# dluvizon/deephar

Hardware: NVIDIA H100
Metric: frames/sec (256x256, 16-frame clips, b32) (higher is better)
Workload: dtype bf16x3 split (fp32 accumulate, wgmma)

## Files before the change

deephar_b200/_ffi.py:

```python
import ctypes as C
import os

_HERE = os.path.dirname(os.path.abspath(__file__))
LIB_PATH = os.environ.get('DEEPHAR_B200_LIB') or os.path.join(_HERE, 'libdeephar_b200.so')


class DeepharB200Error(RuntimeError):
    pass


class dh_view(C.Structure):
    _fields_ = [('p', C.c_void_p), ('n', C.c_int32), ('h', C.c_int32), ('w', C.c_int32),
                ('c', C.c_int32), ('ld', C.c_int32)]


class dh_conv_desc(C.Structure):
    _fields_ = [('kh', C.c_int32), ('kw', C.c_int32), ('sh', C.c_int32), ('sw', C.c_int32),
                ('pad_same', C.c_int32), ('pre_relu', C.c_int32), ('post_relu', C.c_int32),
                ('n_res', C.c_int32),
                ('pre_scale', C.c_void_p), ('pre_shift', C.c_void_p),
                ('post_scale', C.c_void_p), ('post_shift', C.c_void_p),
                ('res', dh_view * 2),
                ('precision', C.c_int32), ('res_up2x', C.c_int32), ('pool_out', dh_view)]


class dh_frame_src(C.Structure):
    _fields_ = [('data', C.c_uint64), ('h', C.c_int32), ('w', C.c_int32), ('stride', C.c_int32),
                ('x0', C.c_int32), ('y0', C.c_int32), ('cw', C.c_int32), ('ch', C.c_int32), ('hflip', C.c_int32),
                ('kx_off', C.c_int32), ('ky_off', C.c_int32), ('kx_coef_off', C.c_int32), ('ky_coef_off', C.c_int32),
                ('ksx', C.c_int32), ('ksy', C.c_int32)]


class dh_packed_w(C.Structure):
    _fields_ = [('hi', C.c_void_p), ('lo', C.c_void_p), ('cout_pad', C.c_int32), ('k', C.c_int32)]


class dh_conv_plan_info(C.Structure):
    _fields_ = [('path', C.c_int32), ('fallback', C.c_int32), ('workspace_bytes', C.c_int64),
                ('n_mtiles', C.c_int32), ('grid_x', C.c_int32), ('grid_y', C.c_int32), ('bn_cta', C.c_int32),
                ('n_kblocks', C.c_int32), ('stages', C.c_int32), ('cluster', C.c_int32), ('bm', C.c_int32),
                ('epi_tma', C.c_int32)]


class dh_clip_window(C.Structure):
    _fields_ = [('src', dh_view), ('dst', dh_view), ('ring', C.c_void_p)]


class dh_jpeg_image(C.Structure):
    _fields_ = [('data', C.c_int64), ('coef', C.c_int64 * 3), ('plane', C.c_int64 * 3), ('out', C.c_int64),
                ('h', C.c_int32), ('w', C.c_int32), ('ncomp', C.c_int32), ('hs', C.c_int32), ('vs', C.c_int32),
                ('mcus_x', C.c_int32), ('mcus_y', C.c_int32), ('bw', C.c_int32 * 3), ('bh', C.c_int32 * 3),
                ('qt', C.c_int32 * 3), ('dc', C.c_int32 * 3), ('ac', C.c_int32 * 3), ('nblocks', C.c_int32),
                ('pad', C.c_int32)]


class dh_jpeg_segment(C.Structure):
    _fields_ = [('begin', C.c_int64), ('end', C.c_int64), ('image', C.c_int32), ('mcu0', C.c_int32),
                ('mcus', C.c_int32), ('pad', C.c_int32)]


class dh_jpeg_huff(C.Structure):
    _fields_ = [('lut', C.c_uint16 * 512), ('maxcode', C.c_int32 * 18), ('valoff', C.c_int32 * 18),
                ('vals', C.c_uint8 * 256)]

# ... 144 lines not shown
```

deephar_b200/csrc/api.cu:

```cuda
#include <stdarg.h>
#include <string.h>
#include "common.cuh"

static thread_local char g_last_error[512] = "";

void dh_set_error(const char* fmt, ...) {
    va_list ap;
    va_start(ap, fmt);
    vsnprintf(g_last_error, sizeof(g_last_error), fmt, ap);
    va_end(ap);
}

extern "C" const char* dh_last_error(void) { return g_last_error; }

extern "C" int dh_version(void) { return 100; }

extern "C" int dh_ctx_create(dh_ctx** out, int device) {
    DH_CHECK_ARG(out != nullptr, "dh_ctx_create: out is NULL");
    int count = 0;
    cudaError_t e = cudaGetDeviceCount(&count);
    if (e != cudaSuccess || count == 0) {
        dh_set_error("dh_ctx_create: no CUDA device (%s) -- this library has no CPU fallback",
                     cudaGetErrorString(e));
        return e == cudaSuccess ? (int)cudaErrorNoDevice : (int)e;
    }
    DH_CHECK_ARG(device >= 0 && device < count, "dh_ctx_create: device %d out of range", device);
    cudaDeviceProp prop;
    e = cudaGetDeviceProperties(&prop, device);
    if (e != cudaSuccess) {
        dh_set_error("cudaGetDeviceProperties: %s", cudaGetErrorString(e));
        return (int)e;
    }
    if (prop.major != 9 || prop.minor != 0) {
        dh_set_error("dh_ctx_create: device %d is sm_%d%d; this build targets sm_90a (H100) only",
                     device, prop.major, prop.minor);
        return -2;
    }
    dh_ctx* c = new dh_ctx();
    c->device = device;
    c->num_sms = prop.multiProcessorCount;
    c->launches = 0;
    c->workspace = nullptr;
    c->workspace_bytes = 0;
    c->last_conv_path = 0;
    c->share_a = 1;
    c->sep_tma = 1;
    c->dbg = 0;
    c->pw_smallk = 1;
    c->dense_patch = 1;
    c->sam3d_stream = 1;
    c->fallbacks = 0;
    c->comm = nullptr;
    c->comm_rank = -1;
    c->comm_world = 0;
    *out = c;
    return 0;
}

extern "C" int dh_comm_destroy(dh_ctx* ctx);

extern "C" int dh_ctx_destroy(dh_ctx* ctx) {
    if (ctx && ctx->comm) dh_comm_destroy(ctx);
    delete ctx;
    return 0;
}

extern "C" int64_t dh_launch_count(dh_ctx* ctx, int reset) {
    if (!ctx) return -1;
    int64_t v = ctx->launches;
    if (reset) ctx->launches = 0;
    return v;
}

extern "C" int dh_set_option(dh_ctx* ctx, const char* name, int value) {
    DH_CHECK_ARG(ctx && name, "dh_set_option: NULL argument");
    if (!strcmp(name, "share_a")) { ctx->share_a = value; return 0; }
    if (!strcmp(name, "sep_tma")) { ctx->sep_tma = value; return 0; }
#ifdef DH_ABLATE
    if (!strcmp(name, "dbg")) { ctx->dbg = value; return 0; }
#endif
    if (!strcmp(name, "pw_smallk")) { ctx->pw_smallk = value; return 0; }
    if (!strcmp(name, "dense_patch")) { ctx->dense_patch = value; return 0; }
    if (!strcmp(name, "sam3d_stream")) { ctx->sam3d_stream = value; return 0; }
    dh_set_error("dh_set_option: unknown option %s", name);
    return -1;
}

extern "C" int dh_last_conv_path(dh_ctx* ctx) { return ctx ? ctx->last_conv_path : -1; }

extern "C" int64_t dh_fallback_count(dh_ctx* ctx, int reset) {
    if (!ctx) return -1;
    int64_t v = ctx->fallbacks;
    if (reset) ctx->fallbacks = 0;
    return v;
}

extern "C" int dh_set_workspace(dh_ctx* ctx, void* ptr, int64_t bytes) {
    DH_CHECK_ARG(ctx != nullptr, "dh_set_workspace: ctx is NULL");
    ctx->workspace = ptr;
    ctx->workspace_bytes = bytes;
// ... 3 lines not shown
```

deephar_b200/csrc/common.cuh:

```cuda
#pragma once
#include <cuda_runtime.h>
#include <stdint.h>
#include <stdio.h>
#include "../../include/deephar_b200.h"

struct dh_ctx {
    int device;
    int num_sms;
    int64_t launches;
    void* workspace;
    int64_t workspace_bytes;
    int last_conv_path;
    int share_a;
    int sep_tma;
    int pw_smallk;
    int sam3d_stream;
    int dense_patch;
    void* comm;
    int comm_rank, comm_world;
    int64_t fallbacks;
    int dbg;
};

void dh_set_error(const char* fmt, ...);

#define DH_CHECK_ARG(cond, ...)            \
    do {                                   \
        if (!(cond)) {                     \
            dh_set_error(__VA_ARGS__);     \
            return -1;                     \
        }                                  \
    } while (0)

#define DH_LAUNCH_EPILOGUE(ctx, nlaunch)                     \
    do {                                                     \
        (ctx)->launches += (nlaunch);                        \
        cudaError_t e__ = cudaGetLastError();                \
// ... 97 lines not shown
```

deephar_b200/csrc/conv_api.cu:

```cuda
#include "tc_common.cuh"

namespace {

struct Choice {
    DhConvPath path;
    bool fallback;
    int64_t workspace_bytes;
    tc::PatchPlan patch;
    tc::SepPlan sep;
    tc::TcPlan tcp;
};

int choose_conv(const dh_ctx* ctx, const ConvParams& p, const dh_packed_w* packed, bool separable, int precision,
                Choice* c) {
    const bool packed_hi = packed && packed->hi;
    c->fallback = false;
    c->workspace_bytes = 0;
    if (separable) {
        DH_CHECK_ARG(!p.pool, "dh_sepconv2d_f32: pool_out is not supported by the separable kernels");
        if (packed_hi && dh_plan_sep_tma(ctx, p, packed, precision, &c->sep)) { c->path = DH_PATH_SEP_TMA; return 0; }
    } else {
        if (!p.up1 && !p.pool && dh_conv_smallk_ok(p)) { c->path = DH_PATH_SIMT; return 0; }
        if (ctx->pw_smallk && !p.up1 && dh_pw_smallk_supported(p)) { c->path = DH_PATH_PW_SMALLK; return 0; }
        DH_CHECK_ARG(!p.pool, "dh_conv2d_f32: pool_out is written by the wide pointwise kernel only (1x1, stride 1, "
// ... 56 lines not shown
    info->n_mtiles = P.n_mtiles;
    info->grid_x = tc::persistent_gx(ctx, pl.gy, P.n_mtiles);
    info->grid_y = pl.gy;
    info->bn_cta = P.bn_cta;
    info->n_kblocks = P.n_kblocks;
    info->cluster = pl.cluster;
    info->bm = tc::BM;
}

int plan_info(const dh_ctx* ctx, const Choice& c, dh_conv_plan_info* info) {
    DH_CHECK_ARG(info, "dh_conv_plan_info: NULL info");
    *info = dh_conv_plan_info{};
    info->path = c.path;
    info->fallback = c.fallback;
    info->workspace_bytes = c.workspace_bytes;
    if (c.path == DH_PATH_TC) {
        tc_info(ctx, c.tcp, c.tcp.k, info);
        info->stages = c.tcp.k.stages;
    }
    if (c.path == DH_PATH_SEP_TMA) {
        tc_info(ctx, c.sep, c.sep.k.t, info);
        info->bm = c.sep.k.bm;
        info->epi_tma = c.sep.k.epi_smem > 0;
    }
    if (c.path == DH_PATH_PATCH) tc_info(ctx, c.patch, c.patch.k.t, info);
    return 0;
}

}

extern "C" int dh_conv2d_f32(dh_ctx* ctx, const dh_view* x, const float* w_hwio,
                             const dh_packed_w* packed, const dh_conv_desc* d, const dh_view* out,
                             void* stream) {
    ConvParams p;
    Choice c;
    int rc = plan_conv(ctx, x, nullptr, w_hwio, packed, d, out, false, &p, &c);
    return rc ? rc : launch_choice(ctx, p, c, false, (cudaStream_t)stream);
}

extern "C" int dh_sepconv2d_f32(dh_ctx* ctx, const dh_view* x, const float* w_dw, const float* w_pw,
                                const dh_packed_w* packed_pw, const dh_conv_desc* d,
                                const dh_view* out, void* stream) {
    ConvParams p;
    Choice c;
    int rc = plan_conv(ctx, x, w_dw, w_pw, packed_pw, d, out, true, &p, &c);
    return rc ? rc : launch_choice(ctx, p, c, true, (cudaStream_t)stream);
// ... 19 lines not shown
```

deephar_b200/csrc/conv_sep.cu:

```cuda
#include "tc_common.cuh"

namespace tcs {
using namespace tc;
using R = tc::Roles<2, 1>;
constexpr int WARP_EPI0 = R::WARP_EPI0, WARP_TMA = R::WARP_TMA, WARP_PATCH = R::WARP_PATCH, NTHREADS = R::NTHREADS,
              REGS_PROD = R::REGS_PROD, REGS_EPI = R::REGS_EPI, REGS_CTRL = R::REGS_CTRL;

constexpr int NWG = 128;
constexpr int NPW = 1;
constexpr int NA = 4;
constexpr int NB = 3;
constexpr int NP = 3;
#ifdef DH_ABLATE
constexpr int DBG_TILE64 = 1 << 14, DBG_TILE128 = 1 << 15;
constexpr int DBG_EPI_REG = 1 << 16;
#endif

template <int TBM, int KS, int TW, bool SHARE, bool BNPRO, bool LO>
__global__ void __launch_bounds__(NTHREADS, 1)
sep_tma_kernel(const __grid_constant__ SepParams SP, const __grid_constant__ CUtensorMap map_hi,
               const __grid_constant__ CUtensorMap map_lo, const __grid_constant__ CUtensorMap map_x,
               const __grid_constant__ CUtensorMap map_out, const __grid_constant__ CUtensorMap map_r0,
               const __grid_constant__ CUtensorMap map_r1) {
    constexpr int PAD = KS / 2;
    constexpr int PC = TW + 2 * PAD;
    constexpr int OR = TBM / 32;
    constexpr int NR = OR + KS - 1;
    constexpr int NC = 4 + KS - 1;
    constexpr int A_BYTES = TBM * 64;
#ifdef DH_ABLATE
    const int DBG = SP.dbg;
#else
    constexpr int DBG = 0;
#endif
    const TcParams& P = SP.t;
    extern __shared__ __align__(1024) uint8_t smem_raw[];
    if (smem_u32(smem_raw) & 1023u) __trap();
    uint8_t* smem = smem_raw;
    const int tid = threadIdx.x;
    const int warp = tid >> 5, lane = tid & 31;
    constexpr bool want_lo = LO;
    const int b_bytes = P.bn_cta * 64;
    uint8_t* b_ring = smem + NA * 2 * A_BYTES;
    uint8_t* patch0 = b_ring + NB * 2 * b_bytes;
    uint8_t* epi_buf = patch0 + NP * SP.patch_stride;
    uint64_t* bars = reinterpret_cast<uint64_t*>(epi_buf + SP.epi_smem);
    float* post = reinterpret_cast<float*>(bars + 64);
    constexpr int NB_A = NA + 2 * NA;
    const uint32_t bar_full0 = smem_u32(bars), bar_empty0 = smem_u32(bars + NA), bar_fullb0 = smem_u32(bars + NB_A),
                   bar_emptyb0 = smem_u32(bars + NB_A + NB), bar_pfull0 = smem_u32(bars + NB_A + 2 * NB),
                   bar_pempty0 = smem_u32(bars + NB_A + 2 * NB + NP), bar_epi_full0 = smem_u32(bars + NB_A + 2 * NB + 2 * NP),
                   bar_epi_empty = bar_epi_full0 + 16;
    const bool epi = TBM == BM64 && SP.epi_smem > 0;
    const int n0 = blockIdx.y * P.bn_cta;
    const int nkb = P.n_kblocks;
    const uint32_t my_rank = SHARE ? cluster_ctarank() : 0u;

    if (warp == WARP_TMA && lane == 0) {
        tma_prefetch_desc(&map_hi);
        if (want_lo) tma_prefetch_desc(&map_lo);
        tma_prefetch_desc(&map_x);
        if (epi) {
            tma_prefetch_desc(&map_out);
            mbar_init(bar_epi_full0, 1);
            mbar_init(bar_epi_full0 + 8, 1);
            mbar_init(bar_epi_empty, 1);
        }
        for (int s = 0; s < NA; ++s) {
            mbar_init(bar_full0 + 8 * s, SHARE ? 1u : (uint32_t)NWG);
            const uint32_t releases = SHARE && (uint32_t)(s & 1) == my_rank ? 2u : 1u;
            mbar_init(bar_empty0 + 16 * s, releases);
            mbar_init(bar_empty0 + 16 * s + 8, releases);
        }
        for (int s = 0; s < NB; ++s) {
            mbar_init(bar_fullb0 + 8 * s, 1);
            mbar_init(bar_emptyb0 + 8 * s, 1);
        }
        for (int s = 0; s < NP; ++s) {
            mbar_init(bar_pfull0 + 8 * s, 1);
            mbar_init(bar_pempty0 + 8 * s, NWG);
        }
        fence_barrier_init();
    }
    if (SHARE) cluster_sync_all(); else __syncthreads();

    const int tiles_mine = ((int)P.n_mtiles - (int)blockIdx.x + (int)gridDim.x - 1) / (int)gridDim.x;
    const int total_g = tiles_mine * nkb;
    const int n_own = SHARE ? (total_g - (int)my_rank + 1) / 2 : total_g;

    if (warp < WARP_EPI0) {
        reg_prod<REGS_PROD, R::LAUNCH_REGS>();
        const ConvParams& c = P.c;
        const int w = warp >> 2;
        const int tw = tid & (NWG - 1);
        const int cp = tw & 15;
        const int blk = tw >> 4;
        constexpr int XB = TW / 4;
        const int strip = blk / XB, xb = blk - strip * XB;
        const int fn = (strip * OR) / SP.ry, ry = (strip * OR) - fn * SP.ry;
        const int prr = SP.ry + 2 * PAD;
        const float* pbase0 = reinterpret_cast<const float*>(patch0) +
                             ((size_t)((fn * prr + ry) * PC + xb * 4)) * SBK + cp * 2;
        const int row0 = strip * OR * TW + xb * 4;
        const float lowb = c.pre_relu ? 0.f : -3.402823466e38f;
        unsigned colmask = 0;
        if (BNPRO) {
#pragma unroll
            for (int q = 0; q < NC; ++q) {
                const int ix = xb * 4 + q - PAD;
                if (ix >= 0 && ix < TW) colmask |= 1u << q;
            }
        }
        float2 wt[KS][KS];
        auto load_taps = [&](int jn) {
            const int gn = SHARE ? 2 * jn + (int)my_rank : jn;
            const int kbn = gn % nkb;
            const float* wp = c.w_dw + kbn * SBK + cp * 2;
#pragma unroll
            for (int a = 0; a < KS; ++a)
#pragma unroll
                for (int b = 0; b < KS; ++b)
                    wt[a][b] = __ldg(reinterpret_cast<const float2*>(wp + (size_t)(a * KS + b) * c.Cin));
        };
        if (w < n_own) load_taps(w);
        for (int j = w; j < n_own; j += NPW) {
            const int pb_i = j % NP;
            const uint32_t pfull = bar_pfull0 + 8 * pb_i, pempty = bar_pempty0 + 8 * pb_i;
            const float* pbase = pbase0 + (size_t)pb_i * (SP.patch_stride / 4);
            const int g = SHARE ? 2 * j + (int)my_rank : j;
            const int ti = g / nkb, kb = g - ti * nkb;
            const int ch = kb * SBK + cp * 2;
            float2 acc[OR][4];
#pragma unroll
            for (int o = 0; o < OR; ++o)
#pragma unroll
                for (int q = 0; q < 4; ++q) acc[o][q] = make_float2(0.f, 0.f);
            float2 ps = make_float2(1.f, 1.f), pb = make_float2(0.f, 0.f);
            unsigned rowmask = 0;
            if (BNPRO) {
                ps = __ldg(reinterpret_cast<const float2*>(c.pre_scale + ch));
                pb = __ldg(reinterpret_cast<const float2*>(c.pre_shift + ch));
                const int t = blockIdx.x + ti * gridDim.x;
                const int y0 = SP.fn > 1 ? 0 : ((t * TBM) / TW) % c.H;
#pragma unroll
                for (int r = 0; r < NR; ++r) {
                    const int iy = y0 + ry + r - PAD;
                    if (iy >= 0 && iy < c.H) rowmask |= 1u << r;
                }
            }

            if (!(DBG & 2)) mbar_wait_relaxed(pfull, (uint32_t)((j / NP) & 1), (DBG & 2048) ? 32u : 0u);
            auto load_row = [&](int r, float2* in) {
#pragma unroll
                for (int q = 0; q < NC; ++q) {
                    float2 v = *reinterpret_cast<const float2*>(pbase + (r * PC + q) * SBK);
                    if (BNPRO) v = ffma2(v, ps, pb);
                    v = make_float2(fmaxf(v.x, lowb), fmaxf(v.y, lowb));
                    if (BNPRO && !(((rowmask >> r) & 1u) && ((colmask >> q) & 1u))) v = make_float2(0.f, 0.f);
                    in[q] = v;
                }
            };
            if (!(DBG & 1)) {
                float2 inb[2][NC];
                load_row(0, inb[0]);
#pragma unroll
                for (int r = 0; r < NR; ++r) {
                    if (r + 1 < NR) load_row(r + 1, inb[(r + 1) & 1]);
                    const float2* in = inb[r & 1];
#pragma unroll
                    for (int kx = 0; kx < KS; ++kx)
#pragma unroll
                        for (int o = 0; o < OR; ++o) {
                            const int ky = r - o;
                            if (ky >= 0 && ky < KS) {
#pragma unroll
                                for (int q = 0; q < 4; ++q) acc[o][q] = ffma2(wt[ky][kx], in[q + kx], acc[o][q]);
                            }
                        }
                }
            }
            if (j + NPW < n_own) load_taps(j + NPW);
            if (!(DBG & 2)) mbar_arrive(pempty);

            const int s = g % NA;
            const uint32_t it = (uint32_t)(g / NA);
            wait_stage_free(bar_empty0, s, it, (DBG & 2048) ? 32u : 0u);
            uint8_t* a_hi = smem + (size_t)s * (2 * A_BYTES);
            uint8_t* a_lo = a_hi + A_BYTES;
#pragma unroll
            for (int o = 0; o < OR; ++o)
#pragma unroll
                for (int q = 0; q < 4; ++q) {
                    uint32_t hi, lo;
                    split2(acc[o][q].x, acc[o][q].y, hi, lo);
                    const uint32_t off = swz64(row0 + o * TW + q, cp * 2);
                    *reinterpret_cast<uint32_t*>(a_hi + off) = hi;
                    if (want_lo) *reinterpret_cast<uint32_t*>(a_lo + off) = lo;
                }
            fence_proxy_async();
            if (SHARE) {
                asm volatile("bar.sync %0, %1;" ::"r"(1 + w), "r"(NWG) : "memory");
                if (tw == 0) {
                    mbar_arrive(bar_full0 + 8 * s);
                    const uint32_t peer = my_rank ^ 1u;
                    const uint32_t peer_full = mapa_peer(bar_full0 + 8 * s, peer);
                    if (!(DBG & 8)) {
                        bulk_s2peer(mapa_peer(smem_u32(a_hi), peer), smem_u32(a_hi), A_BYTES, peer_full);
                        if (want_lo) bulk_s2peer(mapa_peer(smem_u32(a_lo), peer), smem_u32(a_lo), A_BYTES, peer_full);
                    }
                }
            } else {
                mbar_arrive(bar_full0 + 8 * s);
            }
        }
    } else if (warp < WARP_TMA) {
        reg_inc<REGS_EPI>();
        stage_post<R::NEPI, bn_max(TBM)>(P, n0, post, tid - 32 * WARP_EPI0);
        const int wg = (warp - WARP_EPI0) >> 2, wt = tid - 32 * WARP_EPI0 - 128 * wg;
        const EpiSmem es{epi ? reinterpret_cast<float*>(epi_buf) : nullptr,
                         P.c.res1 ? reinterpret_cast<const float*>(epi_buf + EPI_BUF_BYTES) : nullptr, bar_epi_full0,
                         bar_epi_empty, &map_out};
        pp_consumer<SHARE, LO, NA, NB, TBM>(P, wg, wt, n0, tiles_mine, make_desc64(smem_u32(smem)), make_desc64(smem_u32(b_ring)),
                                       bar_full0, bar_empty0, bar_fullb0, bar_emptyb0, my_rank, post, DBG,
                                       es);
    } else {
        reg_dec<REGS_CTRL>();
        if (warp == WARP_TMA) {
            if (lane == 0) {
                const uint32_t tx = (DBG & 16) ? 0u : (uint32_t)(want_lo ? 2 : 1) * (uint32_t)b_bytes;
                const uint32_t tx_a = (DBG & 8) ? 0u : (uint32_t)(want_lo ? 2 : 1) * (uint32_t)A_BYTES;
                for (int g = 0; g < total_g; ++g) {
                    const int ti = g / nkb, kb = g - ti * nkb;
                    const int sb = g % NB;
                    const uint32_t itb = (uint32_t)(g / NB);
                    if (itb >= 1) mbar_wait_relaxed(bar_emptyb0 + 8 * sb, (itb - 1) & 1, (DBG & 2048) ? 64u : 0u);
                    const uint32_t full = bar_fullb0 + 8 * sb;
                    mbar_arrive_expect_tx(full, tx);
                    const uint32_t b_hi = smem_u32(b_ring + (size_t)sb * (2 * b_bytes));
                    const uint32_t b_lo = b_hi + (uint32_t)b_bytes;
                    if (!(DBG & 16)) {
                        tma_load_2d(b_hi, &map_hi, kb * SBK, n0, full);
                        if (want_lo) tma_load_2d(b_lo, &map_lo, kb * SBK, n0, full);
                    }
                    if (SHARE && (uint32_t)(g & 1) != my_rank) {
                        const int sa = g % NA;
                        wait_stage_free(bar_empty0, sa, (uint32_t)(g / NA));
                        mbar_arrive_expect_tx(bar_full0 + 8 * sa, tx_a);
                    }
                }
            }
        } else if (warp == WARP_TMA + 1) {
            if (lane == 0 && epi) {
                const ConvParams& c = P.c;
                const uint32_t tx = (DBG & 32) ? 0u
                                               : (c.res0 ? (uint32_t)EPI_BUF_BYTES : 0u) + (c.res1 ? (uint32_t)EPI_R1_BYTES : 0u);
                for (int ti = 0; ti < tiles_mine; ++ti) {
                    if (ti >= 1) mbar_wait_relaxed(bar_epi_empty, (uint32_t)((ti - 1) & 1), 0u);
                    const int m0 = ((int)blockIdx.x + ti * (int)gridDim.x) * TBM;
                    const uint32_t full = bar_epi_full0 + 8 * (ti & 1);
                    mbar_arrive_expect_tx(full, tx);
                    if (tx) {
                        if (c.res0) tma_load_2d(smem_u32(epi_buf), &map_r0, n0, m0, full);
                        if (c.res1) tma_load_2d(smem_u32(epi_buf + EPI_BUF_BYTES), &map_r1, n0, m0 / 4, full);
                    }
                }
            }
        } else if (warp == WARP_PATCH) {
            if (lane == 0 && !(DBG & 2)) {
                const ConvParams& c = P.c;
                auto coords = [&](int j, int& kb, int& nf, int& y0) {
                    const int g = SHARE ? 2 * j + (int)my_rank : j;
                    const int ti = g / nkb;
                    kb = g - ti * nkb;
                    const int t = blockIdx.x + ti * gridDim.x;
                    const int grow = (t * TBM) / TW;
                    nf = grow / c.H;
                    y0 = grow - nf * c.H;
                };
                for (int j = 0; j < n_own; ++j) {
                    int kb, nf, y0;
                    coords(j, kb, nf, y0);
                    const int w = j % NP;
                    const int pfd = (DBG & 1024) ? 2 : (DBG & 4096) ? 4 : (DBG & 8192) ? 9 : 0;
                    if (pfd && j + pfd < n_own) {
                        int kb2, nf2, y2;
                        coords(j + pfd, kb2, nf2, y2);
                        tma_prefetch_4d(&map_x, kb2 * SBK, -PAD, y2 - PAD, nf2);
                    }
                    mbar_wait_relaxed(bar_pempty0 + 8 * w, (uint32_t)(((j / NP) & 1) ^ 1), (DBG & 2048) ? 64u : 0u);
                    const uint32_t pf = bar_pfull0 + 8 * w;
                    mbar_arrive_expect_tx(pf, (uint32_t)SP.patch_bytes);
                    tma_load_4d(smem_u32(patch0 + (size_t)w * SP.patch_stride), &map_x, kb * SBK, -PAD, y0 - PAD, nf, pf);
                }
            }
        }
    }
    if (SHARE) cluster_sync_all(); else __syncthreads();
}

}

bool dh_plan_sep_tma(const dh_ctx* ctx, const ConvParams& p, const dh_packed_w* packed, int precision, tc::SepPlan* pl) {
    using namespace tc;
    using namespace tcs;
    if (!ctx->sep_tma || !packed->lo || !sep_layer_ok(p, packed)) return false;
    if (!(p.W == 32 || p.W == 16 || p.W == 8)) return false;
    const int tr = BM / p.W;
    if (tr <= p.H ? (p.H % tr) != 0 : (tr % p.H) != 0) return false;
    if ((p.Cin % SBK) != 0 || (p.ldx & 3)) return false;
    int bn64, gy64;
    tile_n(p.Cout, &bn64, &gy64, MAX_BN_CTA64);
    const bool fits64 = ctx->share_a && bn64 == MAX_BN_CTA64 && gy64 % 2 == 0;
    bool t64 = fits64 && p.Cin >= 288;
#ifdef DH_ABLATE
    if (ctx->dbg & DBG_TILE64) t64 = fits64;
    if (ctx->dbg & DBG_TILE128) t64 = false;
#endif
    SepParams& SP = pl->k;
    TcParams& P = SP.t;
    P.c = p;
    P.c.K = p.Cin;
    P.k_pad = packed->k;
    P.n_kblocks = p.Cin / SBK;
    P.precision = (precision == 1) ? 1 : 3;
    P.ks = p.kh;
    P.stages = 2;
    const int pad = p.kh / 2;
#ifdef DH_ABLATE
    SP.dbg = ctx->dbg;
    P.dbg = ctx->dbg;
#else
    SP.dbg = 0;
    P.dbg = 0;
#endif
    auto geometry = [&](int bm) {
        int gy;
        tile_n(p.Cout, &P.bn_cta, &gy, bn_max(bm));
        const int trb = bm / p.W;
        SP.bm = bm;
        P.n_mtiles = (p.M + bm - 1) / bm;
        SP.ry = trb <= p.H ? trb : p.H;
        SP.fn = trb <= p.H ? 1 : trb / p.H;
        SP.patch_bytes = SBK * 4 * (p.W + 2 * pad) * (SP.ry + 2 * pad) * SP.fn;
        SP.patch_stride = (SP.patch_bytes + 1023) / 1024 * 1024;
        pl->smem = (size_t)NA * 2 * (bm * 64) + (size_t)NB * 2 * P.bn_cta * 64 + NP * (size_t)SP.patch_stride + 512 +
                   post_smem(bm);
        pl->gy = gy;
        return pl->smem <= SMEM_LIMIT;
    };
    SP.epi_smem = 0;
    if (!(t64 && geometry(BM64)) && !geometry(BM)) return false;
    bool epi = SP.bm == BM64 && tma_view_ok(p.out, p.ldo) && (!p.res0 || tma_view_ok(p.res0, p.ldr0)) &&
               (!p.res1 || (p.up1 && tma_view_ok(p.res1, p.ldr1)));
#ifdef DH_ABLATE
    if (ctx->dbg & DBG_EPI_REG) epi = false;
#endif
    const int epi_smem = EPI_BUF_BYTES + (p.res1 ? EPI_R1_BYTES : 0);
    if (epi && pl->smem + epi_smem <= SMEM_LIMIT) {
        SP.epi_smem = epi_smem;
        pl->smem += epi_smem;
    }
    pl->w = packed;
    pl->cluster = pl->gy % 2 == 0 && ctx->share_a;
    return true;
}

int dh_launch_sep_tma(const dh_ctx* ctx, const tc::SepPlan& pl, cudaStream_t s) {
    using namespace tc;
    using namespace tcs;
    const TcParams& P = pl.k.t;
    const ConvParams& c = P.c;
    const dh_packed_w* w = pl.w;
    const int pad = P.ks / 2;
    CUtensorMap map_hi, map_lo, map_x, map_out{}, map_r0{}, map_r1{};
    const bool epi = pl.k.epi_smem > 0;
    if (!make_map_w(&map_hi, w->hi, w->k, w->cout_pad, SBK, P.bn_cta) ||
        !make_map_w(&map_lo, w->lo, w->k, w->cout_pad, SBK, P.bn_cta) ||
        !make_map_x(&map_x, c.x, c.ldx, c.Cin, c.W, c.H, c.N, c.W + 2 * pad, pl.k.ry + 2 * pad, pl.k.fn) ||
        (epi && !make_map_rows(&map_out, c.out, c.Cout, c.M, c.ldo, MAX_BN_CTA64, BM64)) ||
        (epi && c.res0 && !make_map_rows(&map_r0, c.res0, c.Cout, c.M, c.ldr0, MAX_BN_CTA64, BM64)) ||
        (epi && c.res1 && !make_map_rows(&map_r1, c.res1, c.Cout, c.M / 4, c.ldr1, MAX_BN_CTA64, BM64 / 4))) {
        dh_set_error("dh_launch_sep_tma: cuTensorMapEncodeTiled failed");
        return -1;
    }
    return pick<5, 3>(P.ks, [&](auto ks) {
        return pick<32, 16, 8>(c.W, [&](auto tw) {
            return pick<true, false>(c.pre_scale != nullptr, [&](auto bnpro) {
                return pick<true, false>(P.precision == 3, [&](auto lo) {
                    if (pl.k.bm == BM64)
                        return launch_persistent<sep_tma_kernel<BM64, ks(), tw(), true, bnpro(), lo()>>(
                            "dh_launch_sep_tma", ctx, pl, P.n_mtiles, NTHREADS, s, map_hi, map_lo, map_x, map_out, map_r0, map_r1);
                    return pick<true, false>(pl.cluster, [&](auto share) {
                        return launch_persistent<sep_tma_kernel<BM, ks(), tw(), share(), bnpro(), lo()>>(
                            "dh_launch_sep_tma", ctx, pl, P.n_mtiles, NTHREADS, s, map_hi, map_lo, map_x, map_out, map_r0, map_r1);
                    });
                });
            });
        });
    });
}
```

deephar_b200/csrc/tc_common.cuh:

```cuda
#pragma once
#include <cuda.h>
#include <cuda_bf16.h>
#include <type_traits>
#include "common.cuh"
#include "conv_params.cuh"

namespace tc {


constexpr int BM = 128;
constexpr int BK = 64;
constexpr int NPROD = 256;
constexpr int MAX_BN_CTA = 96;
constexpr int ACC_N = MAX_BN_CTA / 2;
constexpr int MH = BM / 64;
constexpr int BM64 = 64;
constexpr int MAX_BN_CTA64 = 144;
constexpr int bn_max(int bm) { return bm == BM64 ? MAX_BN_CTA64 : MAX_BN_CTA; }
template <int Q, int NPW = 2>
struct Roles {
    static constexpr int EPQ = Q;
    static constexpr int NEPI = 128 * Q;
    static constexpr int WARP_EPI0 = 4 * NPW;
    static constexpr int WARP_TMA = WARP_EPI0 + 4 * Q, WARP_PATCH = WARP_TMA + 2;
// ... 6 lines not shown
};
constexpr int A_TILE_BYTES = BM * 128;
constexpr int MAX_STAGES = 4;

struct TcParams {
    ConvParams c;
    int n_kblocks;
    int bn_cta;
    int stages;
    int precision;
    int ks;
    int k_pad;
    int n_mtiles;
    int dbg;
};

struct SepParams {
    TcParams t;
    int patch_stride;
    int patch_bytes;
    int ry, fn;
    int bm;
    int epi_smem;
    int dbg;
};

struct PatchParams {
    TcParams t;
    int np, patch_stride, patch_bytes;
    int ntaps, ncb;
    int tw;
    int ry, fn;
    int pc, pr;
    int rows_per_frame;
    int kw;
    int pt, pl, sh, sw;
    int vh, vw;
    int mask;
};

__device__ __forceinline__ void mbar_wait_relaxed(uint32_t bar, uint32_t parity, uint32_t ns) {
    uint32_t ok;
    for (;;) {
        asm volatile(
            "{\n .reg .pred p;\n mbarrier.try_wait.parity.shared::cta.b64 p, [%1], %2;\n selp.u32 %0, 1, 0, p;\n}"
            : "=r"(ok)
// ... 416 lines not shown
                const int g = g0 + kb, s = g % NA, sb = g % NB;
                if (!(dbg & 128)) mbar_wait(bar_full0 + 8 * s, (uint32_t)(g / NA) & 1);
                mbar_wait(bar_fullb0 + 8 * sb, (uint32_t)(g / NB) & 1);
                if (kb == nkb - 1 && ti + 1 < tiles_mine) pp_pass(wg);
                da = dbase + (uint64_t)((uint32_t)s * sta16);
                db = dbase_b + (uint64_t)((uint32_t)sb * stb16);
            },
            [&](int kb) {
                const int g = g0 + kb, s = g % NA;
                const uint32_t producer = (uint32_t)(s & 1);
                wg_release(bar_empty0 + 16 * s + 8 * ((g / NA) & 1), wg, wt, SHARE && producer != rank, producer);
                if (wt == 0) mbar_arrive(bar_emptyb0 + 8 * (g % NB));
            });
        if constexpr (TBM == BM64) {
            if (es.buf) {
                wg_epilogue_smem(P, acc, ti, m0, n0, wg, wt, post, es);
                continue;
            }
        }
        wg_epilogue(P, acc, m0, n0, wt, post);
    }
}

typedef CUresult (*EncodeTiledFn)(CUtensorMap*, CUtensorMapDataType, cuuint32_t, void*, const cuuint64_t*,
                                  const cuuint64_t*, const cuuint32_t*, const cuuint32_t*, CUtensorMapInterleave,
                                  CUtensorMapSwizzle, CUtensorMapL2promotion, CUtensorMapFloatOOBfill);

static inline EncodeTiledFn get_encode() {
    static EncodeTiledFn fn = nullptr;
    if (!fn) {
        void* p = nullptr;
        cudaDriverEntryPointQueryResult qres;
        if (cudaGetDriverEntryPoint("cuTensorMapEncodeTiled", &p, cudaEnableDefault, &qres) == cudaSuccess &&
            qres == cudaDriverEntryPointSuccess)
            fn = (EncodeTiledFn)p;
    }
    return fn;
}

static inline bool make_map_w(CUtensorMap* map, const void* base, int k_pad, int rows, int kblk, int box_rows) {
    EncodeTiledFn enc = get_encode();
    if (!enc) return false;
    cuuint64_t dims[2] = {(cuuint64_t)k_pad, (cuuint64_t)rows};
    cuuint64_t strides[1] = {(cuuint64_t)k_pad * 2};
    cuuint32_t box[2] = {(cuuint32_t)kblk, (cuuint32_t)box_rows};
    cuuint32_t estr[2] = {1, 1};
// ... 124 lines not shown
```

include/deephar_b200.h:

```cpp
#ifndef DEEPHAR_B200_H
#define DEEPHAR_B200_H

#include <stdint.h>

#ifdef __cplusplus
extern "C" {
#endif

typedef struct dh_view {
    float*  p;
    int32_t n, h, w, c;
    int32_t ld;
} dh_view;

typedef struct dh_conv_desc {
    int32_t kh, kw, sh, sw;
    int32_t pad_same;
    int32_t pre_relu;
    int32_t post_relu;
    int32_t n_res;
    const float* pre_scale;
    const float* pre_shift;
    const float* post_scale;
    const float* post_shift;
// ... 23 lines not shown
int dh_tc_k_pad(int k);
int dh_last_conv_path(dh_ctx* ctx);
int64_t dh_fallback_count(dh_ctx* ctx, int reset);

int dh_conv2d_f32(dh_ctx* ctx, const dh_view* x, const float* w_hwio, const dh_packed_w* packed,
                  const dh_conv_desc* d, const dh_view* out, void* stream);

int dh_sepconv2d_f32(dh_ctx* ctx, const dh_view* x, const float* w_dw, const float* w_pw,
                     const dh_packed_w* packed_pw, const dh_conv_desc* d, const dh_view* out,
                     void* stream);

typedef struct dh_conv_plan_info {
    int32_t path;
    int32_t fallback;
    int64_t workspace_bytes;
    int32_t n_mtiles;
    int32_t grid_x, grid_y;
    int32_t bn_cta;
    int32_t n_kblocks;
    int32_t stages;
    int32_t cluster;
    int32_t bm;
    int32_t epi_tma;
} dh_conv_plan_info;
int dh_conv2d_plan(dh_ctx* ctx, const dh_view* x, const float* w_hwio, const dh_packed_w* packed,
                   const dh_conv_desc* d, const dh_view* out, dh_conv_plan_info* info);
int dh_sepconv2d_plan(dh_ctx* ctx, const dh_view* x, const float* w_dw, const float* w_pw,
                      const dh_packed_w* packed_pw, const dh_conv_desc* d, const dh_view* out,
                      dh_conv_plan_info* info);

int dh_maxpool2d_f32(dh_ctx* ctx, const dh_view* x, int kh, int kw, int sh, int sw, int pad_same,
                     const dh_view* out, void* stream);
int dh_upsample2x_add_f32(dh_ctx* ctx, const dh_view* a, const dh_view* b, const dh_view* out,
                          void* stream);
int dh_add_n_f32(dh_ctx* ctx, const dh_view* in, int n_in, const float* scale, const float* shift,
                 int relu, const dh_view* out, void* stream);

int dh_softargmax2d_f32(dh_ctx* ctx, const dh_view* h, const dh_view* d, float alpha,
                        int conf_on_prob, float* out_pose, float* out_conf,
                        const dh_view* prob_out, void* stream);

int dh_softargmax2d_ctx_f32(dh_ctx* ctx, const dh_view* h, int nj, int n_ctx, float alpha_mix,
                            float* out_pose, float* out_vis, void* stream);

int dh_softargmax3d_f32(dh_ctx* ctx, const dh_view* h, int nj, int depth_maps,
                        float* out_pose, float* out_vis, void* stream);
// ... 150 lines not shown
```

Measured before the change: 4063.

## Co-schedule pairs of 64-row tiles in separable conv TMA kernel

Adds a co-scheduled mode to the separable-conv kernel. Each A stage now holds two 64-row M tiles, so the two consumer warpgroups each take one tile of the pair and share a single B-stage fetch. The goal is to halve the B-operand traffic and the per-k-block barrier overhead when there are many k-blocks. In exchange the A ring doubles in size and the patch ring shrinks to two buffers, and the mode is only chosen when there are enough k-blocks and the epilogue TMA views are valid.

Result: faster. 4204, median of 6 (+3.5%).

```diff
diff --git a/deephar_b200/_ffi.py b/deephar_b200/_ffi.py
--- a/deephar_b200/_ffi.py
+++ b/deephar_b200/_ffi.py
@@ -39,7 +39,7 @@
     _fields_ = [('path', C.c_int32), ('fallback', C.c_int32), ('workspace_bytes', C.c_int64),
                 ('n_mtiles', C.c_int32), ('grid_x', C.c_int32), ('grid_y', C.c_int32), ('bn_cta', C.c_int32),
                 ('n_kblocks', C.c_int32), ('stages', C.c_int32), ('cluster', C.c_int32), ('bm', C.c_int32),
-                ('epi_tma', C.c_int32)]
+                ('epi_tma', C.c_int32), ('cosched', C.c_int32)]
 
 
 class dh_clip_window(C.Structure):
diff --git a/deephar_b200/csrc/api.cu b/deephar_b200/csrc/api.cu
--- a/deephar_b200/csrc/api.cu
+++ b/deephar_b200/csrc/api.cu
@@ -45,6 +45,7 @@
     c->last_conv_path = 0;
     c->share_a = 1;
     c->sep_tma = 1;
+    c->sep_cosched = 1;
     c->dbg = 0;
     c->pw_smallk = 1;
     c->dense_patch = 1;
@@ -76,6 +77,7 @@
     DH_CHECK_ARG(ctx && name, "dh_set_option: NULL argument");
     if (!strcmp(name, "share_a")) { ctx->share_a = value; return 0; }
     if (!strcmp(name, "sep_tma")) { ctx->sep_tma = value; return 0; }
+    if (!strcmp(name, "sep_cosched")) { ctx->sep_cosched = value; return 0; }
 #ifdef DH_ABLATE
     if (!strcmp(name, "dbg")) { ctx->dbg = value; return 0; }
 #endif
diff --git a/deephar_b200/csrc/common.cuh b/deephar_b200/csrc/common.cuh
--- a/deephar_b200/csrc/common.cuh
+++ b/deephar_b200/csrc/common.cuh
@@ -13,6 +13,7 @@
     int last_conv_path;
     int share_a;
     int sep_tma;
+    int sep_cosched;
     int pw_smallk;
     int sam3d_stream;
     int dense_patch;
diff --git a/deephar_b200/csrc/conv_api.cu b/deephar_b200/csrc/conv_api.cu
--- a/deephar_b200/csrc/conv_api.cu
+++ b/deephar_b200/csrc/conv_api.cu
@@ -102,6 +102,7 @@
         tc_info(ctx, c.sep, c.sep.k.t, info);
         info->bm = c.sep.k.bm;
         info->epi_tma = c.sep.k.epi_smem > 0;
+        info->cosched = c.sep.k.cosched;
     }
     if (c.path == DH_PATH_PATCH) tc_info(ctx, c.patch, c.patch.k.t, info);
     return 0;
diff --git a/deephar_b200/csrc/conv_sep.cu b/deephar_b200/csrc/conv_sep.cu
--- a/deephar_b200/csrc/conv_sep.cu
+++ b/deephar_b200/csrc/conv_sep.cu
@@ -11,12 +11,18 @@
 constexpr int NA = 4;
 constexpr int NB = 3;
 constexpr int NP = 3;
+constexpr int NP_COS = 2;
+constexpr int COS_PATCH_MAX = SBK * 4 * (32 + 4) * (2 + 4);
+static_assert(NA * 4 * (BM64 * 64) + NB * 2 * (MAX_BN_CTA64 * 64) + NP_COS * COS_PATCH_MAX + EPI_BUF_BYTES +
+                  EPI_R1_BYTES + 512 + post_smem(BM64) <= SMEM_LIMIT,
+              "co-scheduled 64 x 144 rings do not fit at 5x5, W = 32, with an up2x residual");
+constexpr int COS_MIN_KBLOCKS = 12;
 #ifdef DH_ABLATE
 constexpr int DBG_TILE64 = 1 << 14, DBG_TILE128 = 1 << 15;
 constexpr int DBG_EPI_REG = 1 << 16;
 #endif
 
-template <int TBM, int KS, int TW, bool SHARE, bool BNPRO, bool LO>
+template <int TBM, int KS, int TW, bool SHARE, bool BNPRO, bool LO, bool COS>
 __global__ void __launch_bounds__(NTHREADS, 1)
 sep_tma_kernel(const __grid_constant__ SepParams SP, const __grid_constant__ CUtensorMap map_hi,
                const __grid_constant__ CUtensorMap map_lo, const __grid_constant__ CUtensorMap map_x,
@@ -28,6 +34,10 @@
     constexpr int NR = OR + KS - 1;
     constexpr int NC = 4 + KS - 1;
     constexpr int A_BYTES = TBM * 64;
+    static_assert(!COS || (TBM == BM64 && SHARE), "co-scheduling runs the 64-row tiles of cluster pairs");
+    constexpr int NH = COS ? 2 : 1;
+    constexpr int A_STAGE = NH * 2 * A_BYTES;
+    constexpr int NPB = COS ? NP_COS : NP;
 #ifdef DH_ABLATE
     const int DBG = SP.dbg;
 #else
@@ -41,16 +51,16 @@
     const int warp = tid >> 5, lane = tid & 31;
     constexpr bool want_lo = LO;
     const int b_bytes = P.bn_cta * 64;
-    uint8_t* b_ring = smem + NA * 2 * A_BYTES;
+    uint8_t* b_ring = smem + NA * A_STAGE;
     uint8_t* patch0 = b_ring + NB * 2 * b_bytes;
-    uint8_t* epi_buf = patch0 + NP * SP.patch_stride;
+    uint8_t* epi_buf = patch0 + NPB * SP.patch_stride;
     uint64_t* bars = reinterpret_cast<uint64_t*>(epi_buf + SP.epi_smem);
     float* post = reinterpret_cast<float*>(bars + 64);
     constexpr int NB_A = NA + 2 * NA;
     const uint32_t bar_full0 = smem_u32(bars), bar_empty0 = smem_u32(bars + NA), bar_fullb0 = smem_u32(bars + NB_A),
                    bar_emptyb0 = smem_u32(bars + NB_A + NB), bar_pfull0 = smem_u32(bars + NB_A + 2 * NB),
-                   bar_pempty0 = smem_u32(bars + NB_A + 2 * NB + NP), bar_epi_full0 = smem_u32(bars + NB_A + 2 * NB + 2 * NP),
-                   bar_epi_empty = bar_epi_full0 + 16;
+                   bar_pempty0 = smem_u32(bars + NB_A + 2 * NB + NPB),
+                   bar_epi_full0 = smem_u32(bars + NB_A + 2 * NB + 2 * NPB), bar_epi_empty = bar_epi_full0 + 16;
     const bool epi = TBM == BM64 && SP.epi_smem > 0;
     const int n0 = blockIdx.y * P.bn_cta;
     const int nkb = P.n_kblocks;
@@ -68,15 +78,15 @@
         }
         for (int s = 0; s < NA; ++s) {
             mbar_init(bar_full0 + 8 * s, SHARE ? 1u : (uint32_t)NWG);
-            const uint32_t releases = SHARE && (uint32_t)(s & 1) == my_rank ? 2u : 1u;
+            const uint32_t releases = (uint32_t)NH * (SHARE && (uint32_t)(s & 1) == my_rank ? 2u : 1u);
             mbar_init(bar_empty0 + 16 * s, releases);
             mbar_init(bar_empty0 + 16 * s + 8, releases);
         }
         for (int s = 0; s < NB; ++s) {
             mbar_init(bar_fullb0 + 8 * s, 1);
-            mbar_init(bar_emptyb0 + 8 * s, 1);
-        }
-        for (int s = 0; s < NP; ++s) {
+            mbar_init(bar_emptyb0 + 8 * s, NH);
+        }
+        for (int s = 0; s < NPB; ++s) {
             mbar_init(bar_pfull0 + 8 * s, 1);
             mbar_init(bar_pempty0 + 8 * s, NWG);
         }
@@ -85,7 +95,8 @@
     if (SHARE) cluster_sync_all(); else __syncthreads();
 
     const int tiles_mine = ((int)P.n_mtiles - (int)blockIdx.x + (int)gridDim.x - 1) / (int)gridDim.x;
-    const int total_g = tiles_mine * nkb;
+    const int total_g = (COS ? (tiles_mine + 1) / 2 : tiles_mine) * nkb;
+    auto tiles_of = [&](int u) { return COS && 2 * u + 1 < tiles_mine ? 2 : 1; };
     const int n_own = SHARE ? (total_g - (int)my_rank + 1) / 2 : total_g;
 
     if (warp < WARP_EPI0) {
@@ -123,80 +134,87 @@
                     wt[a][b] = __ldg(reinterpret_cast<const float2*>(wp + (size_t)(a * KS + b) * c.Cin));
         };
         if (w < n_own) load_taps(w);
+        int box = 0;
         for (int j = w; j < n_own; j += NPW) {
-            const int pb_i = j % NP;
-            const uint32_t pfull = bar_pfull0 + 8 * pb_i, pempty = bar_pempty0 + 8 * pb_i;
-            const float* pbase = pbase0 + (size_t)pb_i * (SP.patch_stride / 4);
             const int g = SHARE ? 2 * j + (int)my_rank : j;
-            const int ti = g / nkb, kb = g - ti * nkb;
+            const int u = g / nkb, kb = g - u * nkb;
+            const int nh = tiles_of(u);
             const int ch = kb * SBK + cp * 2;
-            float2 acc[OR][4];
-#pragma unroll
-            for (int o = 0; o < OR; ++o)
-#pragma unroll
-                for (int q = 0; q < 4; ++q) acc[o][q] = make_float2(0.f, 0.f);
             float2 ps = make_float2(1.f, 1.f), pb = make_float2(0.f, 0.f);
-            unsigned rowmask = 0;
             if (BNPRO) {
                 ps = __ldg(reinterpret_cast<const float2*>(c.pre_scale + ch));
                 pb = __ldg(reinterpret_cast<const float2*>(c.pre_shift + ch));
-                const int t = blockIdx.x + ti * gridDim.x;
-                const int y0 = SP.fn > 1 ? 0 : ((t * TBM) / TW) % c.H;
-#pragma unroll
-                for (int r = 0; r < NR; ++r) {
-                    const int iy = y0 + ry + r - PAD;
-                    if (iy >= 0 && iy < c.H) rowmask |= 1u << r;
-                }
-            }
-
-            if (!(DBG & 2)) mbar_wait_relaxed(pfull, (uint32_t)((j / NP) & 1), (DBG & 2048) ? 32u : 0u);
-            auto load_row = [&](int r, float2* in) {
-#pragma unroll
-                for (int q = 0; q < NC; ++q) {
-                    float2 v = *reinterpret_cast<const float2*>(pbase + (r * PC + q) * SBK);
-                    if (BNPRO) v = ffma2(v, ps, pb);
-                    v = make_float2(fmaxf(v.x, lowb), fmaxf(v.y, lowb));
-                    if (BNPRO && !(((rowmask >> r) & 1u) && ((colmask >> q) & 1u))) v = make_float2(0.f, 0.f);
-                    in[q] = v;
-                }
-            };
-            if (!(DBG & 1)) {
-                float2 inb[2][NC];
-                load_row(0, inb[0]);
-#pragma unroll
-                for (int r = 0; r < NR; ++r) {
-                    if (r + 1 < NR) load_row(r + 1, inb[(r + 1) & 1]);
-                    const float2* in = inb[r & 1];
-#pragma unroll
-                    for (int kx = 0; kx < KS; ++kx)
-#pragma unroll
-                        for (int o = 0; o < OR; ++o) {
-                            const int ky = r - o;
-                            if (ky >= 0 && ky < KS) {
-#pragma unroll
-                                for (int q = 0; q < 4; ++q) acc[o][q] = ffma2(wt[ky][kx], in[q + kx], acc[o][q]);
+            }
+            const int s = g % NA;
+            uint8_t* a_stage = smem + (size_t)s * A_STAGE;
+            for (int h = 0; h < nh; ++h, ++box) {
+                const int pb_i = box % NPB;
+                const uint32_t pfull = bar_pfull0 + 8 * pb_i, pempty = bar_pempty0 + 8 * pb_i;
+                const float* pbase = pbase0 + (size_t)pb_i * (SP.patch_stride / 4);
+                const int ti = COS ? 2 * u + h : u;
+                float2 acc[OR][4];
+#pragma unroll
+                for (int o = 0; o < OR; ++o)
+#pragma unroll
+                    for (int q = 0; q < 4; ++q) acc[o][q] = make_float2(0.f, 0.f);
+                unsigned rowmask = 0;
+                if (BNPRO) {
+                    const int t = blockIdx.x + ti * gridDim.x;
+                    const int y0 = SP.fn > 1 ? 0 : ((t * TBM) / TW) % c.H;
+#pragma unroll
+                    for (int r = 0; r < NR; ++r) {
+                        const int iy = y0 + ry + r - PAD;
+                        if (iy >= 0 && iy < c.H) rowmask |= 1u << r;
+                    }
+                }
+
+                if (!(DBG & 2)) mbar_wait_relaxed(pfull, (uint32_t)((box / NPB) & 1), (DBG & 2048) ? 32u : 0u);
+                auto load_row = [&](int r, float2* in) {
+#pragma unroll
+                    for (int q = 0; q < NC; ++q) {
+                        float2 v = *reinterpret_cast<const float2*>(pbase + (r * PC + q) * SBK);
+                        if (BNPRO) v = ffma2(v, ps, pb);
+                        v = make_float2(fmaxf(v.x, lowb), fmaxf(v.y, lowb));
+                        if (BNPRO && !(((rowmask >> r) & 1u) && ((colmask >> q) & 1u))) v = make_float2(0.f, 0.f);
+                        in[q] = v;
+                    }
+                };
+                if (!(DBG & 1)) {
+                    float2 inb[2][NC];
+                    load_row(0, inb[0]);
+#pragma unroll
+                    for (int r = 0; r < NR; ++r) {
+                        if (r + 1 < NR) load_row(r + 1, inb[(r + 1) & 1]);
+                        const float2* in = inb[r & 1];
+#pragma unroll
+                        for (int kx = 0; kx < KS; ++kx)
+#pragma unroll
+                            for (int o = 0; o < OR; ++o) {
+                                const int ky = r - o;
+                                if (ky >= 0 && ky < KS) {
+#pragma unroll
+                                    for (int q = 0; q < 4; ++q) acc[o][q] = ffma2(wt[ky][kx], in[q + kx], acc[o][q]);
+                                }
                             }
-                        }
-                }
-            }
-            if (j + NPW < n_own) load_taps(j + NPW);
-            if (!(DBG & 2)) mbar_arrive(pempty);
-
-            const int s = g % NA;
-            const uint32_t it = (uint32_t)(g / NA);
-            wait_stage_free(bar_empty0, s, it, (DBG & 2048) ? 32u : 0u);
-            uint8_t* a_hi = smem + (size_t)s * (2 * A_BYTES);
-            uint8_t* a_lo = a_hi + A_BYTES;
-#pragma unroll
-            for (int o = 0; o < OR; ++o)
-#pragma unroll
-                for (int q = 0; q < 4; ++q) {
-                    uint32_t hi, lo;
-                    split2(acc[o][q].x, acc[o][q].y, hi, lo);
-                    const uint32_t off = swz64(row0 + o * TW + q, cp * 2);
-                    *reinterpret_cast<uint32_t*>(a_hi + off) = hi;
-                    if (want_lo) *reinterpret_cast<uint32_t*>(a_lo + off) = lo;
-                }
+                    }
+                }
+                if (h == nh - 1 && j + NPW < n_own) load_taps(j + NPW);
+                if (!(DBG & 2)) mbar_arrive(pempty);
+
+                if (h == 0) wait_stage_free(bar_empty0, s, (uint32_t)(g / NA), (DBG & 2048) ? 32u : 0u);
+                uint8_t* a_hi = a_stage + h * (2 * A_BYTES);
+                uint8_t* a_lo = a_hi + A_BYTES;
+#pragma unroll
+                for (int o = 0; o < OR; ++o)
+#pragma unroll
+                    for (int q = 0; q < 4; ++q) {
+                        uint32_t hi, lo;
+                        split2(acc[o][q].x, acc[o][q].y, hi, lo);
+                        const uint32_t off = swz64(row0 + o * TW + q, cp * 2);
+                        *reinterpret_cast<uint32_t*>(a_hi + off) = hi;
+                        if (want_lo) *reinterpret_cast<uint32_t*>(a_lo + off) = lo;
+                    }
+            }
             fence_proxy_async();
             if (SHARE) {
                 asm volatile("bar.sync %0, %1;" ::"r"(1 + w), "r"(NWG) : "memory");
@@ -204,9 +222,12 @@
                     mbar_arrive(bar_full0 + 8 * s);
                     const uint32_t peer = my_rank ^ 1u;
                     const uint32_t peer_full = mapa_peer(bar_full0 + 8 * s, peer);
+                    const uint32_t a0 = smem_u32(a_stage);
                     if (!(DBG & 8)) {
-                        bulk_s2peer(mapa_peer(smem_u32(a_hi), peer), smem_u32(a_hi), A_BYTES, peer_full);
-                        if (want_lo) bulk_s2peer(mapa_peer(smem_u32(a_lo), peer), smem_u32(a_lo), A_BYTES, peer_full);
+                        if (want_lo) bulk_s2peer(mapa_peer(a0, peer), a0, (uint32_t)(nh * 2 * A_BYTES), peer_full);
+                        else
+                            for (int h = 0; h < nh; ++h)
+                                bulk_s2peer(mapa_peer(a0 + h * 2 * A_BYTES, peer), a0 + h * 2 * A_BYTES, A_BYTES, peer_full);
                     }
                 }
             } else {
@@ -220,9 +241,14 @@
         const EpiSmem es{epi ? reinterpret_cast<float*>(epi_buf) : nullptr,
                          P.c.res1 ? reinterpret_cast<const float*>(epi_buf + EPI_BUF_BYTES) : nullptr, bar_epi_full0,
                          bar_epi_empty, &map_out};
-        pp_consumer<SHARE, LO, NA, NB, TBM>(P, wg, wt, n0, tiles_mine, make_desc64(smem_u32(smem)), make_desc64(smem_u32(b_ring)),
-                                       bar_full0, bar_empty0, bar_fullb0, bar_emptyb0, my_rank, post, DBG,
-                                       es);
+        if constexpr (COS) {
+            cos_consumer<LO, NA, NB>(P, wg, wt, n0, tiles_mine, make_desc64(smem_u32(smem)), make_desc64(smem_u32(b_ring)),
+                                     bar_full0, bar_empty0, bar_fullb0, bar_emptyb0, my_rank, post, DBG, es);
+        } else {
+            pp_consumer<SHARE, LO, NA, NB, TBM>(P, wg, wt, n0, tiles_mine, make_desc64(smem_u32(smem)),
+                                                make_desc64(smem_u32(b_ring)), bar_full0, bar_empty0, bar_fullb0,
+                                                bar_emptyb0, my_rank, post, DBG, es);
+        }
     } else {
         reg_dec<REGS_CTRL>();
         if (warp == WARP_TMA) {
@@ -230,7 +256,7 @@
                 const uint32_t tx = (DBG & 16) ? 0u : (uint32_t)(want_lo ? 2 : 1) * (uint32_t)b_bytes;
                 const uint32_t tx_a = (DBG & 8) ? 0u : (uint32_t)(want_lo ? 2 : 1) * (uint32_t)A_BYTES;
                 for (int g = 0; g < total_g; ++g) {
-                    const int ti = g / nkb, kb = g - ti * nkb;
+                    const int u = g / nkb, kb = g - u * nkb;
                     const int sb = g % NB;
                     const uint32_t itb = (uint32_t)(g / NB);
                     if (itb >= 1) mbar_wait_relaxed(bar_emptyb0 + 8 * sb, (itb - 1) & 1, (DBG & 2048) ? 64u : 0u);
@@ -245,7 +271,7 @@
                     if (SHARE && (uint32_t)(g & 1) != my_rank) {
                         const int sa = g % NA;
                         wait_stage_free(bar_empty0, sa, (uint32_t)(g / NA));
-                        mbar_arrive_expect_tx(bar_full0 + 8 * sa, tx_a);
+                        mbar_arrive_expect_tx(bar_full0 + 8 * sa, tx_a * (uint32_t)tiles_of(u));
                     }
                 }
             }
@@ -268,29 +294,33 @@
         } else if (warp == WARP_PATCH) {
             if (lane == 0 && !(DBG & 2)) {
                 const ConvParams& c = P.c;
-                auto coords = [&](int j, int& kb, int& nf, int& y0) {
+                auto coords = [&](int j, int h, int& kb, int& nf, int& y0) {
                     const int g = SHARE ? 2 * j + (int)my_rank : j;
-                    const int ti = g / nkb;
-                    kb = g - ti * nkb;
-                    const int t = blockIdx.x + ti * gridDim.x;
+                    const int u = g / nkb;
+                    kb = g - u * nkb;
+                    const int t = blockIdx.x + (COS ? 2 * u + h : u) * gridDim.x;
                     const int grow = (t * TBM) / TW;
                     nf = grow / c.H;
                     y0 = grow - nf * c.H;
                 };
+                int box = 0;
                 for (int j = 0; j < n_own; ++j) {
-                    int kb, nf, y0;
-                    coords(j, kb, nf, y0);
-                    const int w = j % NP;
                     const int pfd = (DBG & 1024) ? 2 : (DBG & 4096) ? 4 : (DBG & 8192) ? 9 : 0;
                     if (pfd && j + pfd < n_own) {
                         int kb2, nf2, y2;
-                        coords(j + pfd, kb2, nf2, y2);
+                        coords(j + pfd, 0, kb2, nf2, y2);
                         tma_prefetch_4d(&map_x, kb2 * SBK, -PAD, y2 - PAD, nf2);
                     }
-                    mbar_wait_relaxed(bar_pempty0 + 8 * w, (uint32_t)(((j / NP) & 1) ^ 1), (DBG & 2048) ? 64u : 0u);
-                    const uint32_t pf = bar_pfull0 + 8 * w;
-                    mbar_arrive_expect_tx(pf, (uint32_t)SP.patch_bytes);
-                    tma_load_4d(smem_u32(patch0 + (size_t)w * SP.patch_stride), &map_x, kb * SBK, -PAD, y0 - PAD, nf, pf);
+                    const int nh = tiles_of((SHARE ? 2 * j + (int)my_rank : j) / nkb);
+                    for (int h = 0; h < nh; ++h, ++box) {
+                        int kb, nf, y0;
+                        coords(j, h, kb, nf, y0);
+                        const int w = box % NPB;
+                        mbar_wait_relaxed(bar_pempty0 + 8 * w, (uint32_t)(((box / NPB) & 1) ^ 1), (DBG & 2048) ? 64u : 0u);
+                        const uint32_t pf = bar_pfull0 + 8 * w;
+                        mbar_arrive_expect_tx(pf, (uint32_t)SP.patch_bytes);
+                        tma_load_4d(smem_u32(patch0 + (size_t)w * SP.patch_stride), &map_x, kb * SBK, -PAD, y0 - PAD, nf, pf);
+                    }
                 }
             }
         }
@@ -333,28 +363,31 @@
     SP.dbg = 0;
     P.dbg = 0;
 #endif
-    auto geometry = [&](int bm) {
+    auto geometry = [&](int bm, bool cos) {
         int gy;
         tile_n(p.Cout, &P.bn_cta, &gy, bn_max(bm));
         const int trb = bm / p.W;
         SP.bm = bm;
+        SP.cosched = cos;
         P.n_mtiles = (p.M + bm - 1) / bm;
         SP.ry = trb <= p.H ? trb : p.H;
         SP.fn = trb <= p.H ? 1 : trb / p.H;
         SP.patch_bytes = SBK * 4 * (p.W + 2 * pad) * (SP.ry + 2 * pad) * SP.fn;
         SP.patch_stride = (SP.patch_bytes + 1023) / 1024 * 1024;
-        pl->smem = (size_t)NA * 2 * (bm * 64) + (size_t)NB * 2 * P.bn_cta * 64 + NP * (size_t)SP.patch_stride + 512 +
-                   post_smem(bm);
+        pl->smem = (size_t)NA * (cos ? 2 : 1) * 2 * (bm * 64) + (size_t)NB * 2 * P.bn_cta * 64 +
+                   (cos ? NP_COS : NP) * (size_t)SP.patch_stride + 512 + post_smem(bm);
         pl->gy = gy;
         return pl->smem <= SMEM_LIMIT;
     };
+    bool epi_views = tma_view_ok(p.out, p.ldo) && (!p.res0 || tma_view_ok(p.res0, p.ldr0)) &&
+                     (!p.res1 || (p.up1 && tma_view_ok(p.res1, p.ldr1)));
+#ifdef DH_ABLATE
+    if (ctx->dbg & DBG_EPI_REG) epi_views = false;
+#endif
+    const bool cos = ctx->sep_cosched == 2 || (ctx->sep_cosched == 1 && P.n_kblocks >= COS_MIN_KBLOCKS && epi_views);
     SP.epi_smem = 0;
-    if (!(t64 && geometry(BM64)) && !geometry(BM)) return false;
-    bool epi = SP.bm == BM64 && tma_view_ok(p.out, p.ldo) && (!p.res0 || tma_view_ok(p.res0, p.ldr0)) &&
-               (!p.res1 || (p.up1 && tma_view_ok(p.res1, p.ldr1)));
-#ifdef DH_ABLATE
-    if (ctx->dbg & DBG_EPI_REG) epi = false;
-#endif
+    if (!(t64 && ((cos && geometry(BM64, true)) || geometry(BM64, false))) && !geometry(BM, false)) return false;
+    const bool epi = SP.bm == BM64 && epi_views;
     const int epi_smem = EPI_BUF_BYTES + (p.res1 ? EPI_R1_BYTES : 0);
     if (epi && pl->smem + epi_smem <= SMEM_LIMIT) {
         SP.epi_smem = epi_smem;
@@ -388,10 +421,13 @@
             return pick<true, false>(c.pre_scale != nullptr, [&](auto bnpro) {
                 return pick<true, false>(P.precision == 3, [&](auto lo) {
                     if (pl.k.bm == BM64)
-                        return launch_persistent<sep_tma_kernel<BM64, ks(), tw(), true, bnpro(), lo()>>(
-                            "dh_launch_sep_tma", ctx, pl, P.n_mtiles, NTHREADS, s, map_hi, map_lo, map_x, map_out, map_r0, map_r1);
+                        return pick<true, false>(pl.k.cosched != 0, [&](auto cos) {
+                            return launch_persistent<sep_tma_kernel<BM64, ks(), tw(), true, bnpro(), lo(), cos()>>(
+                                "dh_launch_sep_tma", ctx, pl, P.n_mtiles, NTHREADS, s, map_hi, map_lo, map_x, map_out,
+                                map_r0, map_r1);
+                        });
                     return pick<true, false>(pl.cluster, [&](auto share) {
-                        return launch_persistent<sep_tma_kernel<BM, ks(), tw(), share(), bnpro(), lo()>>(
+                        return launch_persistent<sep_tma_kernel<BM, ks(), tw(), share(), bnpro(), lo(), false>>(
                             "dh_launch_sep_tma", ctx, pl, P.n_mtiles, NTHREADS, s, map_hi, map_lo, map_x, map_out, map_r0, map_r1);
                     });
                 });
diff --git a/deephar_b200/csrc/tc_common.cuh b/deephar_b200/csrc/tc_common.cuh
--- a/deephar_b200/csrc/tc_common.cuh
+++ b/deephar_b200/csrc/tc_common.cuh
@@ -52,6 +52,7 @@
     int ry, fn;
     int bm;
     int epi_smem;
+    int cosched;
     int dbg;
 };
 
@@ -514,6 +515,44 @@
     }
 }
 
+template <bool LO, int NA, int NB>
+__device__ __forceinline__ void cos_consumer(const TcParams& P, int wg, int wt, int n0, int tiles_mine, uint64_t dbase,
+                                             uint64_t dbase_b, uint32_t bar_full0, uint32_t bar_empty0,
+                                             uint32_t bar_fullb0, uint32_t bar_emptyb0, uint32_t rank, const float* post,
+                                             int dbg, EpiSmem es) {
+    static_assert(NA % 2 == 0, "each A stage has one producing CTA of the pair");
+    const int nkb = P.n_kblocks;
+    const int b_bytes = P.bn_cta * 64;
+    constexpr int a_bytes = BM64 * 64;
+    float acc[1][MAX_BN_CTA64 / 2];
+    const uint32_t sta16 = (4 * a_bytes) >> 4, stb16 = (uint32_t)(2 * b_bytes) >> 4, alo16 = a_bytes >> 4,
+                   blo16 = (uint32_t)b_bytes >> 4;
+    const uint64_t da_wg = dbase + (uint64_t)(wg * ((2 * a_bytes) >> 4));
+    for (int u = 0; 2 * u < tiles_mine; ++u) {
+        const int ti = 2 * u + wg, g0 = u * nkb, m0 = ((int)blockIdx.x + ti * (int)gridDim.x) * BM64;
+        const bool mine = ti < tiles_mine;
+        if (mine && !es.buf) wg_prefetch_res<BM64>(P, m0, n0, wt);
+        wg_tile<SBK / 16, LO>(
+            P.bn_cta, acc, nkb, 0u, alo16, blo16, mine && !(dbg & 64),
+            [&](int kb, uint64_t& da, uint64_t& db) {
+                const int g = g0 + kb, s = g % NA, sb = g % NB;
+                if (!(dbg & 128)) mbar_wait(bar_full0 + 8 * s, (uint32_t)(g / NA) & 1);
+                mbar_wait(bar_fullb0 + 8 * sb, (uint32_t)(g / NB) & 1);
+                da = da_wg + (uint64_t)((uint32_t)s * sta16);
+                db = dbase_b + (uint64_t)((uint32_t)sb * stb16);
+            },
+            [&](int kb) {
+                const int g = g0 + kb, s = g % NA;
+                const uint32_t producer = (uint32_t)(s & 1);
+                wg_release(bar_empty0 + 16 * s + 8 * ((g / NA) & 1), wg, wt, producer != rank, producer);
+                if (wt == 0) mbar_arrive(bar_emptyb0 + 8 * (g % NB));
+            });
+        if (!mine) break;
+        if (es.buf) wg_epilogue_smem(P, acc, ti, m0, n0, wg, wt, post, es);
+        else wg_epilogue(P, acc, m0, n0, wt, post);
+    }
+}
+
 typedef CUresult (*EncodeTiledFn)(CUtensorMap*, CUtensorMapDataType, cuuint32_t, void*, const cuuint64_t*,
                                   const cuuint64_t*, const cuuint32_t*, const cuuint32_t*, CUtensorMapInterleave,
                                   CUtensorMapSwizzle, CUtensorMapL2promotion, CUtensorMapFloatOOBfill);
diff --git a/include/deephar_b200.h b/include/deephar_b200.h
--- a/include/deephar_b200.h
+++ b/include/deephar_b200.h
@@ -69,6 +69,7 @@
     int32_t cluster;
     int32_t bm;
     int32_t epi_tma;
+    int32_t cosched;
 } dh_conv_plan_info;
 int dh_conv2d_plan(dh_ctx* ctx, const dh_view* x, const float* w_hwio, const dh_packed_w* packed,
                    const dh_conv_desc* d, const dh_view* out, dh_conv_plan_info* info);
```
